# NekoImageLand/retto

Measured on AMD Instinct MI355X. Metric: images/sec end-to-end PP-OCRv4 det+rec @960x960, higher is better.
Workload: dtype f32; 1 GPU; C3: PP-OCRv4 mobile det+cls+rec full pipeline, batch=32 pages of 960x960 per GPU, 32 planted lines/page (planted DB map drives box extraction; det net fully executed, checksum 1.46374e+07); pages resident in HBM when the timed region starts; weights=seeded synthetic, PP-OCRv4 mobile shapes, networks=mobile/f32 f32 mobile/f32, parallelism=dp1 (pages sharded, no per-step collective), batches_in_flight=2

## Files before the change

include/retto_hip.h:

```cpp
#ifndef RETTO_HIP_H
#define RETTO_HIP_H

#include <stddef.h>
#include <stdint.h>

#ifdef __cplusplus
extern "C" {
#endif

#define RT_API __attribute__((visibility("default")))

typedef enum rt_status {
  RT_OK = 0,
  RT_ERR_IO = 1,
  RT_ERR_IMAGE = 2,
  RT_ERR_SHAPE = 3,
  RT_ERR_BACKEND = 4,
  RT_ERR_UTF8 = 5,
  RT_ERR_MODEL_NOT_FOUND = 7,
  RT_ERR_INVALID = 8,
  RT_ERR_CAPACITY = 9
} rt_status;

typedef struct rt_model_source {
// ... 111 lines not shown

RT_API int rt_onnx_to_rtwb(int which, const void* onnx, size_t len, void** out, size_t* out_len, char* err, size_t err_cap);
RT_API void rt_buffer_free(void* p);

RT_API int rt_host_cpu_budget(void);
RT_API int rt_decode_image(const void* data, size_t len, uint8_t** rgb, int* h, int* w, char* err, size_t err_cap);
RT_API int rt_run_encoded_batch(rt_session* s, const void* const* files, const size_t* lens, int n_pages,
                                rt_stage_callback cb, void* user, rt_results** out);
RT_API int rt_submit_encoded_batch(rt_session* s, const void* const* files, const size_t* lens, int n_pages, rt_ticket** out);
RT_API int rt_decode_batch(rt_session* s, const void* const* files, const size_t* lens, int n, int* hs, int* ws,
                           uint8_t* const* out, int mem, int* on_device);
RT_API int rt_debug_jpeg_reconstruct(const void* data, size_t len, uint8_t** rgb, int* h, int* w, int* on_device, char* err,
                                     size_t err_cap);
RT_API int rt_parse_dictionary(const void* data, size_t len, char** out, size_t* out_len, int* n_entries, char* err, size_t err_cap);
RT_API int rt_format_f32(float v, char* buf, size_t cap);
RT_API size_t rt_model_manifest(int which, char* buf, size_t cap);

RT_API int rt_rccl_unique_id(void* id, size_t cap, char* err, size_t err_cap);
RT_API int rt_broadcast_blobs(const void* id, int rank, int world, int device_id, int root, int n_blobs, void** data, size_t* lens,
                              char* err, size_t err_cap);

RT_API void rt_debug_set_variants(int gemm_variant, int dw_variant, int flags);
RT_API int rt_debug_conv16(rt_session* s, const float* x, int n, int cin, int h, int w, const float* wt, int cout, int kh, int kw,
                           int sh, int sw, const float* bias, int act, float* out);
RT_API int rt_bench_gemm(rt_session* s, long long M, int K, int N, int variant, int iters, float* ms_out, float* maxdiff_out);
RT_API int rt_bench_gemm_err(rt_session* s, long long M, int K, int N, int variant, int rows, int act, unsigned seed, double* out4);
#define RT_DEBUG_CANARY 0x7FA5C3E1u
RT_API int rt_debug_gemm(rt_session* s, const float* A, long long M, int K, int lda, const float* W, int N, const float* bias,
                         int act, int has_lab, float lab_a, float lab_c, const float* residual, int ld_res, const float* se_scale,
                         int ld_scale, const long long* img_rows, int n_img, int se_rows, int ldc, int coff, int variant, int ctc,
                         float* out, int* idx_out, float* prob_out, int* plan_out);
RT_API int rt_debug_attention(rt_session* s, const float* qkv, long long rows, const int* tokens, int n_lines, int heads,
                              float* out);
RT_API int rt_bench_lc(rt_session* s, int n, int h, int w, int cin, int cout, int stride, int form, int iters, float* ms_out, float* maxdiff_out);

#ifdef __cplusplus
}
#endif
#endif
```

retto_amd/_lib.py:

```python
from __future__ import annotations

import ctypes as C
import os

_HERE = os.path.dirname(os.path.abspath(__file__))
LIB_PATH = os.path.join(_HERE, "libretto_hip.so")

RT_OK = 0
RT_MEM_HOST, RT_MEM_DEVICE, RT_MEM_HOST_MAPS_DEVICE = 0, 1, 2
RT_MAX_INFLIGHT = 8
RT_DTYPE_F32, RT_DTYPE_F16 = 0, 1
STATUS_NAMES = {0: "OK", 1: "IOError", 2: "ImageError", 3: "ShapeError", 4: "BackendError", 5: "Utf8Error",
                7: "ModelNotFoundError", 8: "InvalidArgument", 9: "CapacityError"}


class ModelSource(C.Structure):
    _fields_ = [("path", C.c_char_p), ("data", C.c_void_p), ("len", C.c_size_t)]


class Config(C.Structure):
    _fields_ = [
        ("struct_size", C.c_uint32), ("device_id", C.c_int32),
        ("det", ModelSource), ("cls", ModelSource), ("rec", ModelSource), ("dict", ModelSource),
        ("max_side_len", C.c_int32), ("min_side_len", C.c_int32),
        ("det_limit_side_len", C.c_int32), ("det_limit_type", C.c_int32),
        ("det_mean", C.c_float * 3), ("det_std", C.c_float * 3), ("det_scale", C.c_float),
        ("det_thresh", C.c_float), ("det_box_thresh", C.c_float), ("det_unclip_ratio", C.c_float),
        ("det_min_mini_box_size", C.c_int32), ("det_dilation", C.c_int32),
        ("cls_image_shape", C.c_int32 * 3), ("cls_batch_num", C.c_int32), ("cls_thresh", C.c_float),
        ("rec_image_shape", C.c_int32 * 3), ("rec_batch_num", C.c_int32),
        ("max_boxes_per_page", C.c_int32), ("det_sub_batch", C.c_int32), ("lanes", C.c_int32), ("dtype", C.c_int32),
        ("det_score_mode", C.c_int32), ("rec_return_word_box", C.c_int32),
    ]


class Word(C.Structure):
    _fields_ = [("quad", C.c_float * 8), ("first_token", C.c_int32), ("n_tokens", C.c_int32), ("first_col", C.c_int32),
                ("last_col", C.c_int32), ("kind", C.c_int32)]


EXPORTS = [
    "rt_config_default", "rt_create", "rt_destroy", "rt_last_error", "rt_version",
    "rt_det", "rt_cls", "rt_rec", "rt_rec_ragged", "rt_rec_classes", "rt_model_info",
    "rt_resize_both_dims", "rt_resize_both", "rt_det_input_dims", "rt_det_preprocess", "rt_det_postprocess",
    "rt_crop_dims", "rt_crop_images", "rt_scale_and_clip", "rt_resize_norm_width", "rt_resize_norm_image",
    "rt_ctc_decode",
    "rt_run_batch", "rt_run_batch_stream", "rt_submit_batch", "rt_wait_batch", "rt_host_cpu_budget", "rt_results_free", "rt_results_pages", "rt_results_count", "rt_results_boxes",
    "rt_results_det_scores", "rt_results_cls_labels", "rt_results_cls_scores", "rt_results_rec_scores",
    "rt_results_rec_tokens", "rt_results_rec_text", "rt_results_rec_words", "rt_results_rec_word_text", "rt_debug_word_boxes", "rt_results_det_checksum", "rt_results_json",
    "rt_device_malloc", "rt_device_free", "rt_memcpy_h2d", "rt_memcpy_d2h", "rt_synchronize",
    "rt_set_lanes", "rt_profile_enable", "rt_profile_get",
    "rt_onnx_to_rtwb", "rt_buffer_free", "rt_model_manifest", "rt_decode_image", "rt_run_encoded_batch",
    "rt_submit_encoded_batch", "rt_decode_batch", "rt_debug_jpeg_reconstruct",
    "rt_debug_set_variants", "rt_bench_gemm", "rt_bench_gemm_err", "rt_bench_lc", "rt_debug_conv16", "rt_debug_gemm", "rt_debug_attention", "rt_parse_dictionary", "rt_format_f32", "rt_rccl_unique_id", "rt_broadcast_blobs",
]

STAGE_CALLBACK = C.CFUNCTYPE(None, C.c_void_p, C.c_int, C.c_int, C.c_char_p)

_lib = None


def source_digest() -> str:
    import glob
    import hashlib
    h = hashlib.sha256()
    files = sorted(glob.glob(os.path.join(_HERE, "csrc", "*.hip")) + glob.glob(os.path.join(_HERE, "csrc", "*.cpp")) +
                   glob.glob(os.path.join(_HERE, "csrc", "*.h")) + [os.path.join(os.path.dirname(_HERE), "include", "retto_hip.h")])
    for f in files:
        h.update(os.path.basename(f).encode()); h.update(open(f, "rb").read())
    return h.hexdigest()[:16]


def load():
    global _lib
    if _lib is not None:
        return _lib
    if not os.path.exists(LIB_PATH):
        raise ImportError(
            f"{LIB_PATH} is missing: build it with `make -C retto_amd/csrc` (python -c 'import __graft_entry__ as g; "
            "g.build()'). retto_amd has no CPU fallback.")
    lib = C.CDLL(LIB_PATH)
    P = C.POINTER
    lib.rt_last_error.restype = C.c_char_p
    lib.rt_last_error.argtypes = [C.c_void_p]
    lib.rt_version.restype = C.c_char_p
    lib.rt_create.argtypes = [P(Config), P(C.c_void_p)]
    lib.rt_destroy.argtypes = [C.c_void_p]
# ... 43 lines not shown
                                         C.c_float, C.c_void_p]
    lib.rt_ctc_decode.argtypes = [C.c_void_p, C.c_void_p, C.c_int, C.c_int, C.c_int, C.c_void_p, C.c_void_p,
                                  C.c_void_p, C.c_void_p, C.c_void_p]
    lib.rt_run_batch.argtypes = [C.c_void_p, P(C.c_void_p), P(C.c_int), P(C.c_int), C.c_int, C.c_int, P(C.c_void_p),
                                 P(C.c_void_p)]
    lib.rt_submit_batch.argtypes = [C.c_void_p, P(C.c_void_p), P(C.c_int), P(C.c_int), C.c_int, C.c_int, P(C.c_void_p), P(C.c_void_p)]
    lib.rt_wait_batch.argtypes = [C.c_void_p, C.c_void_p, P(C.c_void_p)]
    lib.rt_run_batch_stream.argtypes = [C.c_void_p, P(C.c_void_p), P(C.c_int), P(C.c_int), C.c_int, C.c_int, P(C.c_void_p),
                                        STAGE_CALLBACK, C.c_void_p, P(C.c_void_p)]
    lib.rt_profile_get.argtypes = [C.c_void_p, P(P(C.c_char_p)), P(P(C.c_float)), P(P(C.c_int)), P(C.c_int)]
    lib.rt_onnx_to_rtwb.argtypes = [C.c_int, C.c_void_p, C.c_size_t, P(C.c_void_p), P(C.c_size_t), C.c_char_p, C.c_size_t]
    lib.rt_buffer_free.argtypes = [C.c_void_p]
    lib.rt_buffer_free.restype = None
    lib.rt_model_manifest.argtypes = [C.c_int, C.c_char_p, C.c_size_t]
    lib.rt_decode_image.argtypes = [C.c_char_p, C.c_size_t, P(C.c_void_p), P(C.c_int), P(C.c_int), C.c_char_p, C.c_size_t]
    lib.rt_run_encoded_batch.argtypes = [C.c_void_p, P(C.c_char_p), P(C.c_size_t), C.c_int, C.c_void_p, C.c_void_p, P(C.c_void_p)]
    lib.rt_submit_encoded_batch.argtypes = [C.c_void_p, P(C.c_char_p), P(C.c_size_t), C.c_int, P(C.c_void_p)]
    lib.rt_decode_batch.argtypes = [C.c_void_p, P(C.c_char_p), P(C.c_size_t), C.c_int, P(C.c_int), P(C.c_int), P(C.c_void_p),
                                    C.c_int, P(C.c_int)]
    lib.rt_debug_jpeg_reconstruct.argtypes = [C.c_char_p, C.c_size_t, P(C.c_void_p), P(C.c_int), P(C.c_int), P(C.c_int),
                                              C.c_char_p, C.c_size_t]
    lib.rt_model_manifest.restype = C.c_size_t
    lib.rt_parse_dictionary.argtypes = [C.c_char_p, C.c_size_t, P(C.c_void_p), P(C.c_size_t), P(C.c_int), C.c_char_p, C.c_size_t]
    lib.rt_results_rec_words.argtypes = [C.c_void_p, C.c_int, C.c_int, P(P(Word))]
    lib.rt_results_rec_word_text.argtypes = [C.c_void_p, C.c_int, C.c_int, C.c_int]
    lib.rt_results_rec_word_text.restype = C.c_char_p
    lib.rt_debug_word_boxes.argtypes = [C.c_char_p, C.c_size_t, P(C.c_int32), P(C.c_int32), C.c_int, C.c_int, C.c_int, C.c_int,
                                        P(C.c_float), C.c_int, C.c_int, C.c_int, C.c_int, C.c_int, P(Word), P(C.c_int)]
    lib.rt_debug_gemm.argtypes = [C.c_void_p, C.c_void_p, C.c_longlong, C.c_int, C.c_int, C.c_void_p, C.c_int, C.c_void_p,
                                  C.c_int, C.c_int, C.c_float, C.c_float, C.c_void_p, C.c_int, C.c_void_p,
                                  C.c_int, C.c_void_p, C.c_int, C.c_int, C.c_int, C.c_int, C.c_int, C.c_int,
                                  C.c_void_p, C.c_void_p, C.c_void_p, C.c_void_p]
    lib.rt_debug_attention.argtypes = [C.c_void_p, C.c_void_p, C.c_longlong, C.c_void_p, C.c_int, C.c_int, C.c_void_p]
    _lib = lib
    return lib
```

retto_amd/csrc/api.cpp:

```cpp
#include <thread>
#include <sched.h>
#include <atomic>
#include <cmath>
#include <cstdio>
#include <cstdlib>
#include <cstring>
#include <new>

#include "geom_math.h"
#include "session.h"
#include "onnx_import.h"
#include "image_decode.h"

using namespace rt;

static thread_local std::string g_create_error;
static void capture_variant_defaults();
const char* rt_results_json_impl(rt_results* r, int page, int stage);

static void quiesce(rt_session* s) {
  if (!s) return;
  (void)hipSetDevice(s->device);
  if (s->st) (void)hipStreamSynchronize(s->st);
  for (auto& h : s->helpers)
// ... 788 lines not shown
      RT_HIP_CHECK(hipMemcpy(idx_out, didx, (size_t)M * sizeof(int), hipMemcpyDeviceToHost));
      RT_HIP_CHECK(hipMemcpy(prob_out, dprob, (size_t)M * sizeof(float), hipMemcpyDeviceToHost));
    }
    plan_out[0] = (int)plan.kernel; plan_out[1] = plan.nt; plan_out[2] = plan.kg; plan_out[3] = plan.se; plan_out[4] = plan.bf;
  });
}

RT_API int rt_debug_attention(rt_session* s, const float* qkv, long long rows, const int* tokens, int n_lines, int heads, float* out) {
  RT_REQUIRE(s && qkv && tokens && out, s, "rt_debug_attention: null argument");
  RT_REQUIRE(rows > 0 && rows < (1ll << 30) && n_lines > 0 && heads > 0 && heads <= 64, s, "rt_debug_attention: bad shape");
  long long total = 0;
  int maxT = 0;
  for (int i = 0; i < n_lines; i++) {
    RT_REQUIRE(tokens[i] > 0, s, "rt_debug_attention: a line without tokens");
    total += tokens[i]; maxT = std::max(maxT, tokens[i]);
  }
  RT_REQUIRE(total == rows, s, "rt_debug_attention: the lines' tokens do not add up to rows");
  return guarded(s, [&] {
    RT_HIP_CHECK(hipSetDevice(s->device));
    const int hd = 15, C = heads * hd;
    std::vector<ImgGeom> geom;
    long long off = 0;
    for (int i = 0; i < n_lines; i++) { geom.push_back(ImgGeom{off, 1, tokens[i], 0}); off += tokens[i]; }
    DevBufs bufs;
    float* dq = bufs.alloc<float>((size_t)rows * 3 * C);
    float* dout = bufs.alloc<float>((size_t)rows * C);
    ImgGeom* dg = bufs.alloc<ImgGeom>(n_lines);
    RT_HIP_CHECK(hipMemcpy(dq, qkv, (size_t)rows * 3 * C * sizeof(float), hipMemcpyHostToDevice));
    RT_HIP_CHECK(hipMemcpy(dg, geom.data(), geom.size() * sizeof(ImgGeom), hipMemcpyHostToDevice));
    RT_HIP_CHECK(hipMemset(dout, 0, (size_t)rows * C * sizeof(float)));
    nn::attention(s->st, dq, dg, n_lines, maxT, heads, hd, dout);
    RT_HIP_CHECK(hipStreamSynchronize(s->st));
    RT_HIP_CHECK(hipMemcpy(out, dout, (size_t)rows * C * sizeof(float), hipMemcpyDeviceToHost));
  });
}

RT_API int rt_bench_lc(rt_session* s, int n, int h, int w, int cin, int cout, int stride, int form, int iters, float* ms_out, float* maxdiff_out) {
  RT_REQUIRE(s && ms_out && n > 0 && h > 0 && w > 0 && (stride == 1 || stride == 2 || stride == 21), s, "rt_bench_lc: bad argument");
  return guarded(s, [&] {
    RT_HIP_CHECK(hipSetDevice(s->device));
    const int Cp = round_up(cin, 4), Np = round_up(cout, 16), ldy = chan_pitch(cout), nkc = (Cp + nn::KC - 1) / nn::KC;
    const int sh = stride == 21 ? 2 : stride, sw = stride == 21 ? 1 : stride;
    const int ho = (h + sh - 1) / sh, wo = (w + sw - 1) / sw;
    std::vector<ImgGeom> gi(n), go(n);
    for (int i = 0; i < n; i++) { gi[i] = ImgGeom{(long long)i * h * w, h, w, 0}; go[i] = ImgGeom{(long long)i * ho * wo, ho, wo, 0}; }
    const size_t nin = (size_t)n * h * w * Cp, nout = (size_t)n * ho * wo * ldy;
    std::vector<float> hx(nin), hwd(9 * Cp), hbd(Cp, 0.05f), hw((size_t)nkc * Np * nn::KC, 0.f), hb(Np, 0.1f);
    uint32_t st = 777;
    auto rnd = [&]() { st = st * 1664525u + 1013904223u; return ((st >> 8) & 0xffff) / 32768.0f - 1.0f; };
    for (auto& v : hx) v = rnd();
    for (auto& v : hwd) v = rnd() * 0.3f;
    for (int k = 0; k < cin; k++) for (int c = 0; c < cout; c++) hw[((size_t)(k / nn::KC) * Np + c) * nn::KC + k % nn::KC] = rnd() * 0.1f;
    DevBufs bufs;
    RestoreInt keep_form(nn::g_lc_wave);
    float *dx = bufs.alloc<float>(nin), *dwd = bufs.alloc<float>(hwd.size()), *dbd = bufs.alloc<float>(hbd.size()), *dw = bufs.alloc<float>(hw.size()),
          *db = bufs.alloc<float>(hb.size()), *dy = bufs.alloc<float>(nout), *dy0 = bufs.alloc<float>(nout);
    ImgGeom *dgi = bufs.alloc<ImgGeom>(n), *dgo = bufs.alloc<ImgGeom>(n);
    RT_HIP_CHECK(hipMemset(dy, 0, nout * 4)); RT_HIP_CHECK(hipMemset(dy0, 0, nout * 4));
    RT_HIP_CHECK(hipMemcpy(dx, hx.data(), nin * 4, hipMemcpyHostToDevice)); RT_HIP_CHECK(hipMemcpy(dwd, hwd.data(), hwd.size() * 4, hipMemcpyHostToDevice));
    RT_HIP_CHECK(hipMemcpy(dbd, hbd.data(), hbd.size() * 4, hipMemcpyHostToDevice)); RT_HIP_CHECK(hipMemcpy(dw, hw.data(), hw.size() * 4, hipMemcpyHostToDevice));
    RT_HIP_CHECK(hipMemcpy(db, hb.data(), hb.size() * 4, hipMemcpyHostToDevice));
    RT_HIP_CHECK(hipMemcpy(dgi, gi.data(), n * sizeof(ImgGeom), hipMemcpyHostToDevice)); RT_HIP_CHECK(hipMemcpy(dgo, go.data(), n * sizeof(ImgGeom), hipMemcpyHostToDevice));
    Epilogue e; e.bias = db; e.act = ACT_HSWISH; e.has_lab = 1; e.lab_a = 1.01f; e.lab_c = 0.02f;
    const int dw_act = (sh == 2 && sw == 2) ? ACT_NONE : ACT_HSWISH, dw_lab = !(sh == 2 && sw == 2);
    float* dy1 = nullptr;
    auto run = [&](float* out) {
// ... 34 lines not shown
```

retto_amd/csrc/nets.cpp:

```cpp
#include "nets.h"
#include "onnx_import.h"

#include <algorithm>
#include <cstdlib>
#include <cstring>

namespace rt {

static void finish_level(Level& L) {
  long long off = 0;
  L.maxH = L.maxW = 0; L.maxPix = 0;
  for (auto& g : L.h) {
    g.off = off; g.pad_ = 0;
    off += (long long)g.H * g.W;
    L.maxH = std::max(L.maxH, g.H); L.maxW = std::max(L.maxW, g.W);
    L.maxPix = std::max(L.maxPix, (long long)g.H * g.W);
  }
  L.total = off;
}
Level make_level(const std::vector<std::pair<int, int>>& hw) {
  Level L;
  for (auto& p : hw) L.h.push_back(ImgGeom{0, p.first, p.second, 0});
  finish_level(L);
  return L;
// ... 503 lines not shown
  for (const LcBlock& b : blocks_) lv.push_back(down_level(lv.back(), b.sh, b.sw));
  Lt = pool_level(lv.back(), 3, 2);
  std::vector<Level*> ups = {&L0};
  for (auto& l : lv) ups.push_back(&l);
  ups.push_back(&Lt);
  upload_levels(c, ups);
  float* t = c.arena->alloc<float>((size_t)lv[0].total * 16);
  { ProfScope ps(c.prof, c.st, "stem");
    nn::stem_conv(c.st, x, L0.d, lv[0].d, lv[0].n(), lv[0].maxH, lv[0].maxW, 16, stem_w_, stem_b_, ACT_NONE, t); }
  for (size_t i = 0; i < blocks_.size(); i++) t = run_lc(c, blocks_[i], t, lv[i], lv[i + 1]);
  const long long rows = Lt.total;
  const int C = 480, D = 120;
  float* cat = c.arena->alloc<float>((size_t)rows * 2 * C);
  { ProfScope ps(c.prof, c.st, "avgpool");
    nn::avgpool_3x2(c.st, t, lv.back().d, Lt.d, Lt.n(), Lt.maxPix, C, cat, 2 * C); }
  float* z1 = c.arena->alloc<float>((size_t)rows * 60);
  unsigned char* tok_flags = nullptr;
  if (nn::conv13_flat_supported(60, conv1_.Npad) && Lt.maxH == 1 && rows > 0) {
    unsigned char* hf = c.pinned->alloc<unsigned char>((size_t)rows);
    memset(hf, 0, (size_t)rows);
    for (const ImgGeom& g : Lt.h)
      if (g.H == 1 && g.W > 0) { hf[g.off] |= 1; hf[g.off + g.W - 1] |= 2; }
    tok_flags = c.arena->alloc<unsigned char>((size_t)rows);
    RT_HIP_CHECK(hipMemcpyAsync(tok_flags, hf, (size_t)rows, hipMemcpyHostToDevice, c.st));
  }
  { ProfScope ps(c.prof, c.st, "conv1x3");
    if (tok_flags) nn::conv13_flat(c.st, cat, 2 * C, rows, tok_flags, C, conv1_.w, 60, conv1_.Npad, z1, 60, make_epi(conv1_, ACT_SWISH));
    else
    nn::conv_sp(c.st, 1, 3, cat, 2 * C, Lt.d, Lt.n(), Lt.maxH, Lt.maxW, C, conv1_.w, 60, conv1_.Npad, z1, 60,
                make_epi(conv1_, ACT_SWISH)); }
  float* z = c.arena->alloc<float>((size_t)rows * D);
  { ProfScope ps(c.prof, c.st, "gemm_neck");
    nn::gemm(c.st, z1, 60, rows, conv2_.K, conv2_.w, D, conv2_.Npad, z, D, 0, make_epi(conv2_, ACT_SWISH)); }
  float* zf = core_.mixer(c, z, Lt);
  { ProfScope ps(c.prof, c.st, "gemm_neck");
    nn::gemm(c.st, zf, D, rows, conv3_.K, conv3_.w, C, conv3_.Npad, cat, 2 * C, C, make_epi(conv3_, ACT_SWISH)); }
  float* z4 = c.arena->alloc<float>((size_t)rows * 60);
  { ProfScope ps(c.prof, c.st, "conv1x3");
    if (tok_flags) nn::conv13_flat(c.st, cat, 2 * C, rows, tok_flags, 2 * C, conv4_.w, 60, conv4_.Npad, z4, 60, make_epi(conv4_, ACT_SWISH));
    else
    nn::conv_sp(c.st, 1, 3, cat, 2 * C, Lt.d, Lt.n(), Lt.maxH, Lt.maxW, 2 * C, conv4_.w, 60, conv4_.Npad, z4, 60,
                make_epi(conv4_, ACT_SWISH)); }
  float* z5 = c.arena->alloc<float>((size_t)rows * D);
  { ProfScope ps(c.prof, c.st, "gemm_neck");
    nn::gemm(c.st, z4, 60, rows, conv1x1_.K, conv1x1_.w, D, conv1x1_.Npad, z5, D, 0, make_epi(conv1x1_, ACT_SWISH)); }
  return core_.head(c, z5, rows, idx_out, prob_out);
}

void SvtrCore::load(WeightStore& ws, const Blob& b, const std::string& prefix) {
  for (int i = 0; i < 2; i++) {
    std::string p = prefix + ".neck.blk" + std::to_string(i);
    blk[i].qkv = pack_linear(ws, b, p + ".qkv", D, 3 * D);
    blk[i].proj = pack_linear(ws, b, p + ".proj", D, D);
    blk[i].fc1 = pack_linear(ws, b, p + ".fc1", D, 2 * D);
    blk[i].fc2 = pack_linear(ws, b, p + ".fc2", 2 * D, D);
    blk[i].n1g = upload_raw(ws, b, p + ".norm1.g", D); blk[i].n1b = upload_raw(ws, b, p + ".norm1.beta", D);
    blk[i].n2g = upload_raw(ws, b, p + ".norm2.g", D); blk[i].n2b = upload_raw(ws, b, p + ".norm2.beta", D);
  }
  ng = upload_raw(ws, b, prefix + ".neck.norm.g", D); nb = upload_raw(ws, b, prefix + ".neck.norm.beta", D);
  const BlobTensor& fw = b.get(prefix + ".head.fc.w");
  if (fw.dims.size() != 2 || fw.dims[0] != D) throw RtError(3, "RTWB: unexpected shape for " + prefix + ".head.fc.w");
  classes = fw.dims[1];
  fc = pack_linear(ws, b, prefix + ".head.fc", D, classes);
}

float* SvtrCore::mixer(RunCtx& c, float* z, const Level& Lt) const {
  const long long rows = Lt.total;
  float* qkv = c.arena->alloc<float>((size_t)rows * 3 * D);
  float* a = c.arena->alloc<float>((size_t)rows * D);
  float* a2 = c.arena->alloc<float>((size_t)rows * D);
  float* m = c.arena->alloc<float>((size_t)rows * 2 * D);
  for (int i = 0; i < 2; i++) {
    const Blk& k = blk[i];
    { ProfScope ps(c.prof, c.st, "gemm_neck");
      nn::gemm(c.st, z, D, rows, k.qkv.K, k.qkv.w, 3 * D, k.qkv.Npad, qkv, 3 * D, 0, make_epi(k.qkv, ACT_NONE)); }
    { ProfScope ps(c.prof, c.st, "attention");
      nn::attention(c.st, qkv, Lt.d, Lt.n(), Lt.maxW * Lt.maxH, 8, D / 8, a); }
    { ProfScope ps(c.prof, c.st, "gemm_neck");
      nn::gemm(c.st, a, D, rows, k.proj.K, k.proj.w, D, k.proj.Npad, a2, D, 0, make_epi(k.proj, ACT_NONE)); }
    float* zn = c.arena->alloc<float>((size_t)rows * D);
    { ProfScope ps(c.prof, c.st, "layernorm");
      nn::add_layernorm(c.st, z, a2, rows, D, k.n1g, k.n1b, 1e-5f, zn); }
    { ProfScope ps(c.prof, c.st, "gemm_neck");
      nn::gemm(c.st, zn, D, rows, k.fc1.K, k.fc1.w, 2 * D, k.fc1.Npad, m, 2 * D, 0, make_epi(k.fc1, ACT_SWISH));
      nn::gemm(c.st, m, 2 * D, rows, k.fc2.K, k.fc2.w, D, k.fc2.Npad, a2, D, 0, make_epi(k.fc2, ACT_NONE)); }
    float* zo = c.arena->alloc<float>((size_t)rows * D);
    { ProfScope ps(c.prof, c.st, "layernorm");
      nn::add_layernorm(c.st, zn, a2, rows, D, k.n2g, k.n2b, 1e-5f, zo); }
    z = zo;
  }
  float* zf = c.arena->alloc<float>((size_t)rows * D);
  { ProfScope ps(c.prof, c.st, "layernorm");
    nn::add_layernorm(c.st, z, nullptr, rows, D, ng, nb, 1e-6f, zf); }
  return zf;
}

float* SvtrCore::head(RunCtx& c, const float* z5, long long rows, int* idx_out, float* prob_out) const {
  if (idx_out) {
    const int tiles = nn::gemm_argmax_tiles(fc.Npad);
    Epilogue e = make_epi(fc, ACT_NONE);
    e.am_max = c.arena->alloc<float>((size_t)rows * tiles);
    e.am_sum = c.arena->alloc<float>((size_t)rows * tiles);
// ... 249 lines not shown
```

retto_amd/csrc/nets.h:

```cpp
#pragma once
#include <memory>
#include <string>
#include <map>
#include <vector>

#include "nn.h"
#include "runtime.h"

namespace rt {

struct Level {
  std::vector<ImgGeom> h;
  const ImgGeom* d = nullptr;
  long long total = 0;
  int maxH = 0, maxW = 0;
  long long maxPix = 0;
  int n() const { return (int)h.size(); }
  mutable std::map<int, const int*> a_tabs;
};

struct RunCtx {
  hipStream_t st;
  Arena* arena;
  Pinned* pinned;
// ... 42 lines not shown

class DetModel {
 public:
  virtual ~DetModel() {}
  virtual float* run(RunCtx& c, const float* x, Level& L0) = 0;
  virtual float* run_u8(RunCtx& c, const nn::U8Page* pages, float scale, const float* mean3, const float* std3, Level& L0) = 0;
  virtual const char* arch() const = 0;
  virtual const char* dtype() const = 0;
  virtual size_t weight_bytes() const = 0;
};
class ClsModel {
 public:
  virtual ~ClsModel() {}
  virtual float* run(RunCtx& c, const float* x, Level& L0) = 0;
  virtual const char* dtype() const = 0;
};
class RecModel {
 public:
  virtual ~RecModel() {}
  virtual int classes() const = 0;
  int logits_ld() const { return round_up(classes(), 4); }
  virtual float* run(RunCtx& c, const float* x, Level& L0, Level& Lt, int* idx_out = nullptr, float* prob_out = nullptr) = 0;
  virtual const char* arch() const = 0;
  virtual const char* dtype() const = 0;
  virtual size_t weight_bytes() const = 0;
};

struct SvtrCore {
  struct Blk { PackedDense qkv, proj, fc1, fc2; float *n1g, *n1b, *n2g, *n2b; } blk[2];
  float *ng = nullptr, *nb = nullptr;
  PackedDense fc;
  int classes = 0, D = 120;
  void load(WeightStore& ws, const Blob& b, const std::string& prefix);
  float* mixer(RunCtx& c, float* z, const Level& Lt) const;
  float* head(RunCtx& c, const float* z5, long long rows, int* idx_out, float* prob_out) const;
};

class DetNet : public DetModel {
 public:
  explicit DetNet(const Blob& b);
  float* run(RunCtx& c, const float* x, Level& L0) override { return run(c, x, L0, nullptr, 0.f, nullptr, nullptr); }
  float* run_u8(RunCtx& c, const nn::U8Page* pages, float scale, const float* mean3, const float* std3, Level& L0) override {
    return run(c, nullptr, L0, pages, scale, mean3, std3);
  }
  const char* arch() const override { return "mobile"; }
  const char* dtype() const override { return "f32"; }
  size_t weight_bytes() const override { return ws_.bytes(); }
 private:
  float* run(RunCtx& c, const float* x, Level& L0, const nn::U8Page* pages, float scale, const float* mean3, const float* std3);
  WeightStore ws_;
  float* stem_w_; float* stem_b_;
  std::vector<LcBlock> blocks_;
  int tap_after_[4];
  PackedDense out_[4], ins_[4], inp_[4], head_conv1_;
  float* ins_lin_[4];
  bool has_bias_[4] = {false, false, false, false};
  SeW ins_se_[4], inp_se_[4];
  float *dc1_w_, *dc1_b_, *dc2_w_, *dc2_b_;
  float *head_wf_ = nullptr, *head_wc_ = nullptr, *head_cls4_ = nullptr, *head_cls5_ = nullptr;
  float *inp_wc_[2] = {nullptr, nullptr}, *inp_wm_[2] = {nullptr, nullptr};
};

class RecNet : public RecModel {
 public:
  explicit RecNet(const Blob& b);
  int classes() const override { return core_.classes; }
  float* run(RunCtx& c, const float* x, Level& L0, Level& Lt, int* idx_out = nullptr, float* prob_out = nullptr) override;
// ... 27 lines not shown
```

retto_amd/csrc/nn.h:

```cpp
#pragma once
#include "common.h"
#include "gemm_plan.h"

namespace rt {
namespace nn {

constexpr int KC = 32;

void gemm(hipStream_t st, const float* A, int lda, long long M, int K, const float* Wp, int N, int Npad16, float* C,
          int ldc, int coff, const Epilogue& epi);
void gemm(hipStream_t st, const GemmPlan& p, const float* A, int lda, long long M, int K, const float* Wp, int N, int Npad16,
          float* C, int ldc, int coff, const Epilogue& epi);
void gemm_w(hipStream_t st, const float* A, int lda, long long M, int K, const float* Wp, int N, int Npad16, float* C, int ldc, int coff,
            const Epilogue& epi);
void gemm_dma(hipStream_t st, const float* A, int lda, long long M, int K, const float* Wp, int N, int Npad16, float* C,
              int ldc, int coff, const Epilogue& epi);
void gemm_split(hipStream_t st, const float* A, int lda, long long M, int K, const float* Wp, int N, int Npad16, float* C,
                int ldc, int coff, const Epilogue& epi);
void gemm_split_forget(const float* Wp);
extern int g_dw_sweep;

bool conv13_flat_supported(int N, int Npad16);
void conv13_flat(hipStream_t st, const float* x, int ldx, long long rows, const unsigned char* flags, int Cin, const float* Wp, int N,
                 int Npad16, float* y, int ldy, const Epilogue& epi);
// ... 62 lines not shown
  const float* fine_scale = nullptr; int ld_fs = 0;
  const float* Wf = nullptr; long long wf_img = 0;
  const float* coarse = nullptr; int ld_coarse = 0;
  const float* coarse_scale = nullptr; int ld_cs = 0;
  const float* Wc = nullptr;
  const float* G = nullptr; const ImgGeom* gg = nullptr;
  long long g_plane = 0;
  const float* bias = nullptr;
  float* y = nullptr; int ldy = 0;
  float* pool = nullptr; int pool_tiles = 0;
  int act = ACT_NONE;
};
extern int g_fpn_phase_off;
bool fpn_phase_supported(int cf, int cc);
void fpn_phase(hipStream_t st, const FpnPhaseArgs& a, int cf, int cc, const ImgGeom* gf, const ImgGeom* gc, int n_img, int maxH, int maxW);
void fpn_class(hipStream_t st, const float* z, int ldz, const float* scale, int ld_s, const ImgGeom* geom, int n_img,
               long long max_pix, const float* Wcls, const float* bias, const float* lower, const ImgGeom* glow, long long low_plane,
               float* V, long long plane);
void fpn_compose(hipStream_t st, const float* Wlat, int cin, int C, const float* scale, const float* Wm, int cf, int n_img, float* out);
void se_fc_from_tiles(hipStream_t st, const float* partial, const ImgGeom* geom, int n_img, int tiles_alloc, int C, int Cp,
                      const float* w1, const float* b1, const float* w2, const float* b2, int Cr, float slope, int residual,
                      float* scale);
void db_head_tail(hipStream_t st, const float* x, const ImgGeom* gin, const ImgGeom* gout, int n_img, long long max_pix,
                  const float* w1, const float* b1, const float* w2, const float* b2, float* out);

void avgpool_3x2(hipStream_t st, const float* x, const ImgGeom* gin, const ImgGeom* gout, int n_img, long long max_pix,
                 int Cp, float* y, int ldy);
void maxpool_2x2(hipStream_t st, const float* x, const ImgGeom* gin, const ImgGeom* gout, int n_img, long long max_pix,
                 int Cp, float* y);
void add_layernorm(hipStream_t st, const float* x, const float* r, long long rows, int C, const float* g,
                   const float* beta, float eps, float* y);
void attention(hipStream_t st, const float* qkv, const ImgGeom* geom, int n_img, int maxT, int heads, int hd,
               float* out);
void copy_channels(hipStream_t st, const float* src, int lds, long long rows, int C, float* dst, int ldd, int coff);
void softmax_rows(hipStream_t st, const float* in, int ld, long long rows, int C, float* out);
void argmax_prob_rows(hipStream_t st, const float* in, int ld, long long rows, int C, int* idx, float* prob);
void argmax_rows(hipStream_t st, const float* in, int ld, long long rows, int C, int* idx, float* maxval);

}
}
```

Baseline: 1225 images/s.

## Fuse SVTR mixer proj/LN/MLP/LN/conv3 chain into one row-resident kernel

Adds a fused HIP kernel that runs the per-row chain of the SVTR mixer block (proj GEMM, residual add plus LayerNorm, fc1 with swish, fc2, add plus LayerNorm, and optionally the final LayerNorm and conv3 with swish) with each row kept in registers. Weights stream through a double-buffered LDS ring into MFMA instructions. This replaces several GEMM and layernorm launches and their intermediate HBM round trips in the rec neck. It is on by default, can be turned off with an env var, and adds a debug entry point for comparing against the unfused path. It risks lower occupancy from the heavy register use, and the per-block weight restreaming costs bandwidth.

```diff
diff --git a/include/retto_hip.h b/include/retto_hip.h
--- a/include/retto_hip.h
+++ b/include/retto_hip.h
@@ -167,6 +167,9 @@
                          float* out, int* idx_out, float* prob_out, int* plan_out);
 RT_API int rt_debug_attention(rt_session* s, const float* qkv, long long rows, const int* tokens, int n_lines, int heads,
                               float* out);
+RT_API int rt_debug_svtr_rowchain(rt_session* s, const float* a, const float* z, long long rows, const float* const* w,
+                                  const float* const* b, const float* const* ln, int fused, int ldc, int coff, float* out,
+                                  float* mid_out);
 RT_API int rt_bench_lc(rt_session* s, int n, int h, int w, int cin, int cout, int stride, int form, int iters, float* ms_out, float* maxdiff_out);
 
 #ifdef __cplusplus
diff --git a/retto_amd/_lib.py b/retto_amd/_lib.py
--- a/retto_amd/_lib.py
+++ b/retto_amd/_lib.py
@@ -52,7 +52,7 @@
     "rt_set_lanes", "rt_profile_enable", "rt_profile_get",
     "rt_onnx_to_rtwb", "rt_buffer_free", "rt_model_manifest", "rt_decode_image", "rt_run_encoded_batch",
     "rt_submit_encoded_batch", "rt_decode_batch", "rt_debug_jpeg_reconstruct",
-    "rt_debug_set_variants", "rt_bench_gemm", "rt_bench_gemm_err", "rt_bench_lc", "rt_debug_conv16", "rt_debug_gemm", "rt_debug_attention", "rt_parse_dictionary", "rt_format_f32", "rt_rccl_unique_id", "rt_broadcast_blobs",
+    "rt_debug_set_variants", "rt_bench_gemm", "rt_bench_gemm_err", "rt_bench_lc", "rt_debug_conv16", "rt_debug_gemm", "rt_debug_attention", "rt_debug_svtr_rowchain", "rt_parse_dictionary", "rt_format_f32", "rt_rccl_unique_id", "rt_broadcast_blobs",
 ]
 
 STAGE_CALLBACK = C.CFUNCTYPE(None, C.c_void_p, C.c_int, C.c_int, C.c_char_p)
@@ -162,5 +162,7 @@
                                   C.c_int, C.c_void_p, C.c_int, C.c_int, C.c_int, C.c_int, C.c_int, C.c_int,
                                   C.c_void_p, C.c_void_p, C.c_void_p, C.c_void_p]
     lib.rt_debug_attention.argtypes = [C.c_void_p, C.c_void_p, C.c_longlong, C.c_void_p, C.c_int, C.c_int, C.c_void_p]
+    lib.rt_debug_svtr_rowchain.argtypes = [C.c_void_p, C.c_void_p, C.c_void_p, C.c_longlong, P(C.c_void_p), P(C.c_void_p), P(C.c_void_p),
+                                           C.c_int, C.c_int, C.c_int, C.c_void_p, C.c_void_p]
     _lib = lib
     return lib
diff --git a/retto_amd/csrc/api.cpp b/retto_amd/csrc/api.cpp
--- a/retto_amd/csrc/api.cpp
+++ b/retto_amd/csrc/api.cpp
@@ -844,6 +844,67 @@
     nn::attention(s->st, dq, dg, n_lines, maxT, heads, hd, dout);
     RT_HIP_CHECK(hipStreamSynchronize(s->st));
     RT_HIP_CHECK(hipMemcpy(out, dout, (size_t)rows * C * sizeof(float), hipMemcpyDeviceToHost));
+  });
+}
+
+RT_API int rt_debug_svtr_rowchain(rt_session* s, const float* a, const float* z, long long rows, const float* const* w,
+                                  const float* const* b, const float* const* ln, int fused, int ldc, int coff, float* out, float* mid_out) {
+  RT_REQUIRE(s && a && z && w && b && ln && out, s, "rt_debug_svtr_rowchain: null argument");
+  for (int i = 0; i < 3; i++) RT_REQUIRE(w[i] && b[i], s, "rt_debug_svtr_rowchain: null weight");
+  for (int i = 0; i < 4; i++) RT_REQUIRE(ln[i], s, "rt_debug_svtr_rowchain: null LayerNorm parameter");
+  const bool tail = w[3] != nullptr;
+  RT_REQUIRE(!tail || (b[3] && ln[4] && ln[5]), s, "rt_debug_svtr_rowchain: conv3 needs its bias and the final LayerNorm");
+  const int D = 120, N = tail ? 4 * D : D;
+  RT_REQUIRE(rows > 0 && rows < (1ll << 30) && coff >= 0 && coff % 4 == 0 && ldc % 4 == 0 && ldc >= coff + N && (tail || (ldc == D && coff == 0)),
+             s, "rt_debug_svtr_rowchain: bad shape");
+  return guarded(s, [&] {
+    RT_HIP_CHECK(hipSetDevice(s->device));
+    WeightStore ws;
+    const PackedDense proj = pack_linear(ws, w[0], b[0], D, D), fc1 = pack_linear(ws, w[1], b[1], D, 2 * D),
+                      fc2 = pack_linear(ws, w[2], b[2], 2 * D, D);
+    PackedDense c3;
+    if (tail) c3 = pack_linear(ws, w[3], b[3], D, 4 * D);
+    float* dln[6] = {};
+    for (int i = 0; i < (tail ? 6 : 4); i++) dln[i] = ws.upload(std::vector<float>(ln[i], ln[i] + D));
+    DevBufs bufs;
+    float *da = bufs.alloc<float>((size_t)rows * D), *dz = bufs.alloc<float>((size_t)rows * D);
+    RT_HIP_CHECK(hipMemcpy(da, a, (size_t)rows * D * sizeof(float), hipMemcpyHostToDevice));
+    RT_HIP_CHECK(hipMemcpy(dz, z, (size_t)rows * D * sizeof(float), hipMemcpyHostToDevice));
+    const size_t out_n = (size_t)(rows + 64) * ldc;
+    float* dC = bufs.alloc<float>(out_n);
+    RT_HIP_CHECK(hipMemsetD32Async((hipDeviceptr_t)dC, (int)RT_DEBUG_CANARY, out_n, s->st));
+    float* dzf = nullptr;
+    if (fused) {
+      nn::SvtrRowChain rc;
+      rc.D = D;
+      rc.Wproj = proj.w; rc.bproj = proj.b; rc.proj_K = proj.K; rc.proj_Npad = proj.Npad;
+      rc.Wfc1 = fc1.w; rc.bfc1 = fc1.b; rc.fc1_K = fc1.K; rc.fc1_N = fc1.N; rc.fc1_Npad = fc1.Npad;
+      rc.Wfc2 = fc2.w; rc.bfc2 = fc2.b; rc.fc2_K = fc2.K; rc.fc2_Npad = fc2.Npad;
+      rc.n1g = dln[0]; rc.n1b = dln[1]; rc.n2g = dln[2]; rc.n2b = dln[3]; rc.eps = 1e-5f;
+      if (tail) {
+        rc.ng = dln[4]; rc.nb = dln[5]; rc.eps_f = 1e-6f;
+        rc.W3 = c3.w; rc.b3 = c3.b; rc.c3_K = c3.K; rc.c3_N = c3.N; rc.c3_Npad = c3.Npad;
+      }
+      nn::svtr_rowchain(s->st, da, dz, rows, rc, dC, ldc, coff);
+    } else {
+      float *a2 = bufs.alloc<float>((size_t)rows * D), *zn = bufs.alloc<float>((size_t)rows * D), *m = bufs.alloc<float>((size_t)rows * 2 * D);
+      nn::gemm(s->st, da, D, rows, proj.K, proj.w, D, proj.Npad, a2, D, 0, make_epi(proj, ACT_NONE));
+      nn::add_layernorm(s->st, dz, a2, rows, D, dln[0], dln[1], 1e-5f, zn);
+      nn::gemm(s->st, zn, D, rows, fc1.K, fc1.w, 2 * D, fc1.Npad, m, 2 * D, 0, make_epi(fc1, ACT_SWISH));
+      nn::gemm(s->st, m, 2 * D, rows, fc2.K, fc2.w, D, fc2.Npad, a2, D, 0, make_epi(fc2, ACT_NONE));
+      if (!tail) {
+        nn::add_layernorm(s->st, zn, a2, rows, D, dln[2], dln[3], 1e-5f, dC);
+      } else {
+        float* zo = bufs.alloc<float>((size_t)rows * D);
+        dzf = bufs.alloc<float>((size_t)rows * D);
+        nn::add_layernorm(s->st, zn, a2, rows, D, dln[2], dln[3], 1e-5f, zo);
+        nn::add_layernorm(s->st, zo, nullptr, rows, D, dln[4], dln[5], 1e-6f, dzf);
+        nn::gemm(s->st, dzf, D, rows, c3.K, c3.w, 4 * D, c3.Npad, dC, ldc, coff, make_epi(c3, ACT_SWISH));
+      }
+    }
+    RT_HIP_CHECK(hipStreamSynchronize(s->st));
+    RT_HIP_CHECK(hipMemcpy(out, dC, out_n * sizeof(float), hipMemcpyDeviceToHost));
+    if (mid_out && dzf) RT_HIP_CHECK(hipMemcpy(mid_out, dzf, (size_t)rows * D * sizeof(float), hipMemcpyDeviceToHost));
   });
 }
 
diff --git a/retto_amd/csrc/nets.cpp b/retto_amd/csrc/nets.cpp
--- a/retto_amd/csrc/nets.cpp
+++ b/retto_amd/csrc/nets.cpp
@@ -559,8 +559,9 @@
   float* z = c.arena->alloc<float>((size_t)rows * D);
   { ProfScope ps(c.prof, c.st, "gemm_neck");
     nn::gemm(c.st, z1, 60, rows, conv2_.K, conv2_.w, D, conv2_.Npad, z, D, 0, make_epi(conv2_, ACT_SWISH)); }
-  float* zf = core_.mixer(c, z, Lt);
-  { ProfScope ps(c.prof, c.st, "gemm_neck");
+  float* zf = core_.mixer(c, z, Lt, &conv3_, cat, 2 * C, C);
+  if (zf) {
+    ProfScope ps(c.prof, c.st, "gemm_neck");
     nn::gemm(c.st, zf, D, rows, conv3_.K, conv3_.w, C, conv3_.Npad, cat, 2 * C, C, make_epi(conv3_, ACT_SWISH)); }
   float* z4 = c.arena->alloc<float>((size_t)rows * 60);
   { ProfScope ps(c.prof, c.st, "conv1x3");
@@ -591,10 +592,36 @@
   fc = pack_linear(ws, b, prefix + ".head.fc", D, classes);
 }
 
-float* SvtrCore::mixer(RunCtx& c, float* z, const Level& Lt) const {
+float* SvtrCore::mixer(RunCtx& c, float* z, const Level& Lt, const PackedDense* conv3, float* cat, int ldc, int coff) const {
   const long long rows = Lt.total;
   float* qkv = c.arena->alloc<float>((size_t)rows * 3 * D);
   float* a = c.arena->alloc<float>((size_t)rows * D);
+  if (conv3 && nn::g_svtr_fused) {
+    for (int i = 0; i < 2; i++) {
+      const Blk& k = blk[i];
+      { ProfScope ps(c.prof, c.st, "gemm_neck");
+        nn::gemm(c.st, z, D, rows, k.qkv.K, k.qkv.w, 3 * D, k.qkv.Npad, qkv, 3 * D, 0, make_epi(k.qkv, ACT_NONE)); }
+      { ProfScope ps(c.prof, c.st, "attention");
+        nn::attention(c.st, qkv, Lt.d, Lt.n(), Lt.maxW * Lt.maxH, 8, D / 8, a); }
+      nn::SvtrRowChain rc;
+      rc.D = D;
+      rc.Wproj = k.proj.w; rc.bproj = k.proj.b; rc.proj_K = k.proj.K; rc.proj_Npad = k.proj.Npad;
+      rc.Wfc1 = k.fc1.w; rc.bfc1 = k.fc1.b; rc.fc1_K = k.fc1.K; rc.fc1_N = k.fc1.N; rc.fc1_Npad = k.fc1.Npad;
+      rc.Wfc2 = k.fc2.w; rc.bfc2 = k.fc2.b; rc.fc2_K = k.fc2.K; rc.fc2_Npad = k.fc2.Npad;
+      rc.n1g = k.n1g; rc.n1b = k.n1b; rc.n2g = k.n2g; rc.n2b = k.n2b; rc.eps = 1e-5f;
+      ProfScope ps(c.prof, c.st, "gemm_neck", shape_str(rows, D, i == 0 ? 5 * D : 9 * D, i));
+      if (i == 0) {
+        float* zo = c.arena->alloc<float>((size_t)rows * D);
+        nn::svtr_rowchain(c.st, a, z, rows, rc, zo, D, 0);
+        z = zo;
+      } else {
+        rc.ng = ng; rc.nb = nb; rc.eps_f = 1e-6f;
+        rc.W3 = conv3->w; rc.b3 = conv3->b; rc.c3_K = conv3->K; rc.c3_N = conv3->N; rc.c3_Npad = conv3->Npad;
+        nn::svtr_rowchain(c.st, a, z, rows, rc, cat, ldc, coff);
+      }
+    }
+    return nullptr;
+  }
   float* a2 = c.arena->alloc<float>((size_t)rows * D);
   float* m = c.arena->alloc<float>((size_t)rows * 2 * D);
   for (int i = 0; i < 2; i++) {
diff --git a/retto_amd/csrc/nets.h b/retto_amd/csrc/nets.h
--- a/retto_amd/csrc/nets.h
+++ b/retto_amd/csrc/nets.h
@@ -98,7 +98,8 @@
   PackedDense fc;
   int classes = 0, D = 120;
   void load(WeightStore& ws, const Blob& b, const std::string& prefix);
-  float* mixer(RunCtx& c, float* z, const Level& Lt) const;
+  float* mixer(RunCtx& c, float* z, const Level& Lt, const PackedDense* conv3 = nullptr, float* cat = nullptr, int ldc = 0,
+               int coff = 0) const;
   float* head(RunCtx& c, const float* z5, long long rows, int* idx_out, float* prob_out) const;
 };
 
diff --git a/retto_amd/csrc/nn.h b/retto_amd/csrc/nn.h
--- a/retto_amd/csrc/nn.h
+++ b/retto_amd/csrc/nn.h
@@ -118,6 +118,20 @@
                    const float* beta, float eps, float* y);
 void attention(hipStream_t st, const float* qkv, const ImgGeom* geom, int n_img, int maxT, int heads, int hd,
                float* out);
+struct SvtrRowChain {
+  int D = 0;
+  const float *Wproj = nullptr, *bproj = nullptr; int proj_K = 0, proj_Npad = 0;
+  const float *Wfc1 = nullptr, *bfc1 = nullptr; int fc1_K = 0, fc1_N = 0, fc1_Npad = 0;
+  const float *Wfc2 = nullptr, *bfc2 = nullptr; int fc2_K = 0, fc2_Npad = 0;
+  const float *n1g = nullptr, *n1b = nullptr, *n2g = nullptr, *n2b = nullptr;
+  float eps = 0.f;
+  const float *ng = nullptr, *nb = nullptr;
+  float eps_f = 0.f;
+  const float *W3 = nullptr, *b3 = nullptr; int c3_K = 0, c3_N = 0, c3_Npad = 0;
+};
+extern int g_svtr_fused;
+bool svtr_rowchain_supported(const SvtrRowChain& c);
+void svtr_rowchain(hipStream_t st, const float* a, const float* z, long long rows, const SvtrRowChain& c, float* out, int ldc, int coff);
 void copy_channels(hipStream_t st, const float* src, int lds, long long rows, int C, float* dst, int ldd, int coff);
 void softmax_rows(hipStream_t st, const float* in, int ld, long long rows, int C, float* out);
 void argmax_prob_rows(hipStream_t st, const float* in, int ld, long long rows, int C, int* idx, float* prob);
diff --git a/retto_amd/csrc/nn_svtr.hip b/retto_amd/csrc/nn_svtr.hip
--- /dev/null
+++ b/retto_amd/csrc/nn_svtr.hip
@@ -0,0 +1,271 @@
+#include "nn.h"
+#include "nn_dev.h"
+
+#include <cstdlib>
+
+namespace rt {
+namespace nn {
+
+int g_svtr_fused = getenv("RT_SVTR_FUSED") ? atoi(getenv("RT_SVTR_FUSED")) : 1;
+
+namespace {
+
+constexpr int LROW = KC + 4;
+constexpr int RC_D = 120;
+constexpr int RC_WAVES = 8, RC_THREADS = 64 * RC_WAVES, RC_ROWS = 16 * RC_WAVES;
+constexpr int RC_UCOLS = 128;
+constexpr int RC_USL = 1;
+constexpr int RC_SLAB = RC_UCOLS * LROW;
+constexpr int RC_UNIT = RC_USL * RC_SLAB;
+constexpr int RC_WLD = RC_UCOLS * 8 / RC_THREADS;
+constexpr int RC_MAXU = 36;
+constexpr int RC_STAGES = 4;
+
+struct RowChainArgs {
+  const float* a;
+  const float* z;
+  long long M;
+  const float* W[RC_STAGES];
+  int Npad[RC_STAGES], nkc[RC_STAGES];
+  const float *b_proj, *b_fc1, *b_fc2, *b_c3;
+  const float *n1g, *n1b, *n2g, *n2b, *ng, *nb;
+  float eps, eps_f;
+  float* out;
+  int ldc, coff;
+};
+
+struct Unit { const float* src; int nrows; int slab_stride; };
+
+__device__ __forceinline__ float ln_tree(const float (&p)[4][4]) {
+  float p2[4];
+#pragma unroll
+  for (int j = 0; j < 4; j++) p2[j] = (p[0][j] + p[2][j]) + (p[1][j] + p[3][j]);
+#pragma unroll
+  for (int j = 0; j < 4; j++) p2[j] += __shfl_xor(p2[j], 32);
+#pragma unroll
+  for (int j = 0; j < 4; j++) p2[j] += __shfl_xor(p2[j], 16);
+  return (p2[0] + p2[2]) + (p2[1] + p2[3]);
+}
+__device__ __forceinline__ void ln_rows(const f32x4 (&t)[8], int q, int C, const float* __restrict__ g,
+                                        const float* __restrict__ beta, float eps, f32x4 (&y)[8]) {
+  float p[4][4];
+#pragma unroll
+  for (int nt = 0; nt < 4; nt++) {
+    const bool hi = (nt + 4) * 16 + 4 * q < C;
+#pragma unroll
+    for (int j = 0; j < 4; j++) p[nt][j] = (0.f + t[nt][j]) + (hi ? t[nt + 4][j] : 0.f);
+  }
+  const float mean = ln_tree(p) / (float)C;
+#pragma unroll
+  for (int nt = 0; nt < 4; nt++) {
+    const bool hi = (nt + 4) * 16 + 4 * q < C;
+#pragma unroll
+    for (int j = 0; j < 4; j++) {
+      const float d0 = t[nt][j] - mean;
+      float ss = fmaf(d0, d0, 0.f);
+      if (hi) { const float d1 = t[nt + 4][j] - mean; ss = fmaf(d1, d1, ss); }
+      p[nt][j] = ss;
+    }
+  }
+  const float rstd = 1.0f / sqrtf(ln_tree(p) / (float)C + eps);
+#pragma unroll
+  for (int nt = 0; nt < 8; nt++) {
+    const int col = nt * 16 + 4 * q;
+    y[nt] = f32x4{0.f, 0.f, 0.f, 0.f};
+    if (col < C) {
+      const f32x4 gv = *reinterpret_cast<const f32x4*>(g + col), bv = *reinterpret_cast<const f32x4*>(beta + col);
+#pragma unroll
+      for (int j = 0; j < 4; j++) y[nt][j] = fmaf((t[nt][j] - mean) * rstd, gv[j], bv[j]);
+    }
+  }
+}
+
+struct Ring {
+  float* lds;
+  const Unit* units;
+  int nu, u, tid;
+  f32x4 pw[RC_USL * RC_WLD];
+  __device__ __forceinline__ void fetch(int n) {
+    const Unit d = units[n];
+#pragma unroll
+    for (int sl = 0; sl < RC_USL; sl++)
+#pragma unroll
+      for (int i = 0; i < RC_WLD; i++) {
+        const int idx = tid + RC_THREADS * i, row = min(idx >> 3, d.nrows - 1), c4 = idx & 7;
+        pw[sl * RC_WLD + i] = *reinterpret_cast<const f32x4*>(d.src + sl * d.slab_stride + row * KC + c4 * 4);
+      }
+  }
+  __device__ __forceinline__ void stash(int n) {
+    float* ws = lds + (n & 1) * RC_UNIT;
+#pragma unroll
+    for (int sl = 0; sl < RC_USL; sl++)
+#pragma unroll
+      for (int i = 0; i < RC_WLD; i++) {
+        const int idx = tid + RC_THREADS * i;
+        *reinterpret_cast<f32x4*>(ws + sl * RC_SLAB + (idx >> 3) * LROW + (idx & 7) * 4) = pw[sl * RC_WLD + i];
+      }
+  }
+  template <int NG, int NT>
+  __device__ __forceinline__ void pass(const f32x4 (&a)[NG], f32x4 (&acc)[NT], int r, int q) {
+    static_assert(NG % (2 * RC_USL) == 0, "whole units");
+#pragma unroll
+    for (int nt = 0; nt < NT; nt++) acc[nt] = f32x4{0.f, 0.f, 0.f, 0.f};
+#pragma unroll
+    for (int ku = 0; ku < NG / (2 * RC_USL); ku++) {
+      const bool more = u + 1 < nu;
+      if (more) fetch(u + 1);
+      const float* ws = lds + (u & 1) * RC_UNIT + r * LROW + 4 * q;
+#pragma unroll
+      for (int g2 = 0; g2 < 2 * RC_USL; g2++) {
+        f32x4 b[NT];
+#pragma unroll
+        for (int nt = 0; nt < NT; nt++) b[nt] = *reinterpret_cast<const f32x4*>(ws + (g2 >> 1) * RC_SLAB + nt * 16 * LROW + (g2 & 1) * 16);
+#pragma unroll
+        for (int s = 0; s < 4; s++)
+#pragma unroll
+          for (int nt = 0; nt < NT; nt++)
+            acc[nt] = __builtin_amdgcn_mfma_f32_16x16x4f32(b[nt][s], a[ku * 2 * RC_USL + g2][s], acc[nt], 0, 0, 0);
+      }
+      if (more) stash(u + 1);
+      __syncthreads();
+      u++;
+    }
+  }
+};
+
+template <int ACT, int NT>
+__device__ __forceinline__ void bias_act(const f32x4 (&acc)[NT], const float* __restrict__ bias, int col0, int q, int N, f32x4* o) {
+#pragma unroll
+  for (int nt = 0; nt < NT; nt++) {
+    const int col = col0 + nt * 16 + 4 * q;
+    o[nt] = f32x4{0.f, 0.f, 0.f, 0.f};
+    if (col < N) {
+      const f32x4 bv = *reinterpret_cast<const f32x4*>(bias + col);
+#pragma unroll
+      for (int j = 0; j < 4; j++) o[nt][j] = epi_val<ACT, 0>(acc[nt][j] + bv[j], ACT, 0, 1.f, 0.f);
+    }
+  }
+}
+
+template <int TAIL>
+__global__ __launch_bounds__(RC_THREADS) void k_svtr_rowchain(const RowChainArgs p) {
+  __shared__ __attribute__((aligned(16))) float lds[2 * RC_UNIT];
+  __shared__ Unit units[RC_MAXU];
+  const int tid = threadIdx.x, lane = tid & 63, wave = tid >> 6, r = lane & 15, q = lane >> 4;
+  const int stages = TAIL ? 4 : 3;
+  int nu = 0;
+  auto stage_units = [&](int s) { return (p.Npad[s] + RC_UCOLS - 1) / RC_UCOLS * (p.nkc[s] / RC_USL); };
+  for (int s = 0; s < stages; s++) nu += stage_units(s);
+  if (tid < nu) {
+    int u = tid, s = 0;
+    while (u >= stage_units(s)) { u -= stage_units(s); s++; }
+    const int upp = p.nkc[s] / RC_USL, cp = u / upp, kc = (u % upp) * RC_USL;
+    units[tid].src = p.W[s] + ((long long)kc * p.Npad[s] + cp * RC_UCOLS) * KC;
+    units[tid].nrows = min(RC_UCOLS, p.Npad[s] - cp * RC_UCOLS);
+    units[tid].slab_stride = p.Npad[s] * KC;
+  }
+  __syncthreads();
+  Ring ring{lds, units, nu, 0, tid, {}};
+  ring.fetch(0);
+
+  const long long row = (long long)blockIdx.x * RC_ROWS + wave * 16 + r;
+  const bool live = row < p.M;
+  f32x4 av[8];
+#pragma unroll
+  for (int g = 0; g < 8; g++) {
+    const int col = g * 16 + 4 * q;
+    av[g] = f32x4{0.f, 0.f, 0.f, 0.f};
+    if (live && col < RC_D) av[g] = *reinterpret_cast<const f32x4*>(p.a + row * RC_D + col);
+  }
+  ring.stash(0);
+  __syncthreads();
+
+  f32x4 acc[8], t[8], zn[8];
+  ring.pass<8, 8>(av, acc, r, q);
+  bias_act<ACT_NONE, 8>(acc, p.b_proj, 0, q, RC_D, t);
+#pragma unroll
+  for (int nt = 0; nt < 8; nt++) {
+    const int col = nt * 16 + 4 * q;
+    if (live && col < RC_D) t[nt] = *reinterpret_cast<const f32x4*>(p.z + row * RC_D + col) + t[nt];
+  }
+  ln_rows(t, q, RC_D, p.n1g, p.n1b, p.eps, zn);
+  f32x4 m[16];
+  ring.pass<8, 8>(zn, acc, r, q);
+  bias_act<ACT_SWISH, 8>(acc, p.b_fc1, 0, q, 2 * RC_D, m);
+  {
+    f32x4 acc7[7];
+    ring.pass<8, 7>(zn, acc7, r, q);
+    bias_act<ACT_SWISH, 7>(acc7, p.b_fc1, 128, q, 2 * RC_D, m + 8);
+  }
+  m[15] = f32x4{0.f, 0.f, 0.f, 0.f};
+  ring.pass<16, 8>(m, acc, r, q);
+  bias_act<ACT_NONE, 8>(acc, p.b_fc2, 0, q, RC_D, t);
+#pragma unroll
+  for (int nt = 0; nt < 8; nt++) t[nt] = zn[nt] + t[nt];
+  ln_rows(t, q, RC_D, p.n2g, p.n2b, p.eps, zn);
+  if (TAIL == 0) {
+    if (live) {
+#pragma unroll
+      for (int nt = 0; nt < 8; nt++) {
+        const int col = nt * 16 + 4 * q;
+        if (col < RC_D) *reinterpret_cast<f32x4*>(p.out + row * RC_D + col) = zn[nt];
+      }
+    }
+    return;
+  }
+#pragma unroll
+  for (int nt = 0; nt < 8; nt++) t[nt] = zn[nt];
+  ln_rows(t, q, RC_D, p.ng, p.nb, p.eps_f, zn);
+  float* yrow = p.out + row * p.ldc + p.coff;
+#pragma unroll
+  for (int cp = 0; cp < 3; cp++) {
+    ring.pass<8, 8>(zn, acc, r, q);
+    bias_act<ACT_SWISH, 8>(acc, p.b_c3, cp * 128, q, 4 * RC_D, t);
+    if (live) {
+#pragma unroll
+      for (int nt = 0; nt < 8; nt++) *reinterpret_cast<f32x4*>(yrow + cp * 128 + nt * 16 + 4 * q) = t[nt];
+    }
+  }
+  {
+    f32x4 acc6[6];
+    ring.pass<8, 6>(zn, acc6, r, q);
+    bias_act<ACT_SWISH, 6>(acc6, p.b_c3, 384, q, 4 * RC_D, t);
+    if (live) {
+#pragma unroll
+      for (int nt = 0; nt < 6; nt++) *reinterpret_cast<f32x4*>(yrow + 384 + nt * 16 + 4 * q) = t[nt];
+    }
+  }
+}
+
+}
+
+bool svtr_rowchain_supported(const SvtrRowChain& c) {
+  if (c.D != RC_D || c.proj_K != RC_D || c.proj_Npad != 128 || c.fc1_K != RC_D || c.fc1_N != 2 * RC_D || c.fc1_Npad != 2 * RC_D ||
+      c.fc2_K != 2 * RC_D || c.fc2_Npad != 128)
+    return false;
+  if (c.W3 && (!c.ng || c.c3_K != RC_D || c.c3_N != 4 * RC_D || c.c3_Npad != 4 * RC_D)) return false;
+  return true;
+}
+
+void svtr_rowchain(hipStream_t st, const float* a, const float* z, long long rows, const SvtrRowChain& c, float* out, int ldc,
+                   int coff) {
+  if (rows <= 0) return;
+  const int tail = c.W3 ? 1 : 0;
+  if (!svtr_rowchain_supported(c) || (tail && ((ldc & 3) || (coff & 3)))) throw RtError(8, "svtr_rowchain: unsupported block shape");
+  RowChainArgs p = {};
+  p.a = a; p.z = z; p.M = rows;
+  p.W[0] = c.Wproj; p.Npad[0] = 128; p.nkc[0] = 4;
+  p.W[1] = c.Wfc1; p.Npad[1] = 240; p.nkc[1] = 4;
+  p.W[2] = c.Wfc2; p.Npad[2] = 128; p.nkc[2] = 8;
+  p.W[3] = c.W3; p.Npad[3] = 480; p.nkc[3] = 4;
+  p.b_proj = c.bproj; p.b_fc1 = c.bfc1; p.b_fc2 = c.bfc2; p.b_c3 = c.b3;
+  p.n1g = c.n1g; p.n1b = c.n1b; p.n2g = c.n2g; p.n2b = c.n2b; p.ng = c.ng; p.nb = c.nb;
+  p.eps = c.eps; p.eps_f = c.eps_f;
+  p.out = out; p.ldc = ldc; p.coff = coff;
+  const dim3 grid((unsigned)((rows + RC_ROWS - 1) / RC_ROWS)), block(RC_THREADS);
+  if (tail) RT_LAUNCH(k_svtr_rowchain<1>, grid, block, 0, st, p);
+  else RT_LAUNCH(k_svtr_rowchain<0>, grid, block, 0, st, p);
+}
+
+}
+}
```

Result: no change. 1232 images/s (median of 3 runs) (+0.6%).
